# mkocabas/EpipolarPose

Measured on NVIDIA H100. Metric: multi-view samples/sec (4-view 256x256, bs32), higher is better.
Workload: dtype f16x3 (fp32 operands split into two fp16 planes, 3-pass error-compensated wgmma f16, f32 accumulate: fp32-grade results)

## Files before the change

### epipolarpose_b200/_lib.py

```python
import ctypes
import os

HERE = os.path.dirname(os.path.abspath(__file__))
LIB_PATH = os.environ.get("EPB_LIB_PATH") or os.path.join(HERE, "libepb.so")

EPB_MAX_TAPS = 64
EPB_JPEG_DESC_BYTES = 8192
EPB_JPEG_PLAN_LEN = 10
EPB_JPEG_EVENTS = 6
EPB_JPEG_STATS = 7

c_int, c_i64, c_f, c_d, c_p = (ctypes.c_int, ctypes.c_int64, ctypes.c_float,
                               ctypes.c_double, ctypes.c_void_p)


class ConvGeom(ctypes.Structure):
    _fields_ = [("N", c_int), ("Hi", c_int), ("Wi", c_int), ("Cin", c_int),
                ("Ho", c_int), ("Wo", c_int), ("Cout", c_int),
                ("Hp", c_int), ("Wp", c_int),
                ("os", c_int), ("ph", c_int), ("pw", c_int), ("is_", c_int),
                ("T", c_int),
                ("dh", c_int * EPB_MAX_TAPS), ("dw", c_int * EPB_MAX_TAPS),
                ("wt", c_int * EPB_MAX_TAPS), ("Tw", c_int),
                ("in_relu", c_int), ("accumulate", c_int), ("precision", c_int)]
# ... 25 lines not shown
    "epb_softargmax_fwd": (c_int, [c_p, c_int, c_int, c_int, c_int, c_int, c_int, c_p, c_p, c_p]),
    "epb_softargmax_bwd": (c_int, [c_p, c_int, c_int, c_int, c_int, c_int, c_int, c_p, c_p, c_p, c_p, c_p]),
    "epb_jointloss_fwd_bwd": (c_int, [c_p, c_p, c_p, c_int, c_int, c_int, c_f, c_p, c_p, c_p]),
    "epb_heatmap_joint_loss": (c_int, [c_p, c_p, c_p, c_int, c_int, c_f, c_p, c_p, c_p, c_int, c_int, c_f, c_f,
                                       c_p, c_p, c_p, c_p]),
    "epb_argmax2d": (c_int, [c_p, c_int, c_int, c_int, c_p, c_p, c_p, c_p]),
    "epb_final_preds": (c_int, [c_p, c_int, c_int, c_int, c_int, c_p, c_p, c_int, c_p, c_p, c_p]),
    "epb_patch_to_image": (c_int, [c_p, c_p, c_int, c_int, c_d, c_d, c_d, c_p, c_p]),
    "epb_triangulate": (c_int, [c_p, c_p, c_int, c_p, c_p, c_int, c_int, c_int, c_d, c_p, c_p, c_p]),
    "epb_triangulate_nview": (c_int, [c_p, c_int, c_p, c_int, c_int, c_int, c_p, c_p, c_p]),
    "epb_relative_pose": (c_int, [c_p, c_int, c_p, c_p, c_int, c_int, c_d, c_p, c_p, c_p, c_p, c_p, c_p,
                                  c_p]),
    "epb_project_labels": (c_int, [c_p, c_p, c_p, c_int, c_int, c_d, c_d, c_d, c_p, c_p, c_p]),
    "epb_h36m_eval": (c_int, [c_p, c_p, c_p, c_int, c_int, c_int, ctypes.c_uint32, c_d, c_p, c_p, c_p, c_p, c_p]),
    "epb_pose_normalize": (c_int, [c_p, c_p, c_int, c_int, c_int, c_p, c_p]),
    "epb_kmeans_workspace": (c_int, [c_int, c_int, c_int, ctypes.POINTER(c_i64)]),
    "epb_kmeans_fit": (c_int, [c_p, c_int, c_int, c_int, ctypes.c_uint64, c_int, c_int, c_p, c_p, c_p, c_p, c_p,
                               c_i64, ctypes.POINTER(c_d), ctypes.POINTER(ctypes.c_int32), c_p]),
    "epb_kmeans_assign": (c_int, [c_p, c_int, c_int, c_p, c_int, c_p, c_p, c_p]),
    "epb_add3": (c_int, [c_p, c_p, c_p, c_p, c_i64, c_p]),
    "epb_mask_scale": (c_int, [c_p, c_p, c_f, c_p, c_i64, c_p]),
    "epb_patch_sample": (c_int, [c_p, c_p, c_p, c_p, c_p, c_p, c_p, c_int, c_int, c_int, c_p, c_p, c_p]),
    "epb_patch_sample_occ": (c_int, [c_p] * 7 + [c_int, c_int, c_int] + [c_p] * 5 + [c_p]),
    "epb_patch_joints": (c_int, [c_p, c_p, c_p, c_int, c_int, c_d, c_d, c_d, c_int, c_p, c_p]),
    "epb_bn_finalize_scale": (c_int, [c_p, c_i64, c_int, c_p, c_p, c_f, c_f] + [c_p] * 12),
    "epb_softargmax_bwd_split": (c_int, [c_p] + [c_int] * 5 + [c_p] * 7),
    "epb_softargmax_flip_fwd": (c_int, [c_p] + [c_int] * 5 + [ctypes.POINTER(c_int), c_int, c_p, c_p]),
    "epb_act_scale": (c_int, [c_p, c_p, c_p, c_i64, c_int, c_p, c_p, c_p, c_p, c_p, c_p]),
    "epb_bn_act_split": (c_int, [c_p] * 8 + [c_int, c_i64, c_int, c_p, c_p, c_p, c_p]),
    "epb_bn_relu_maxpool_split": (c_int, [c_p] * 6 + [c_int] * 4 + [c_p]),
    "epb_im2col_split": (c_int, [c_p] * 3 + [c_int] * 11 + [c_p]),
    "epb_split16": (c_int, [c_p, ctypes.c_longlong, c_p, c_p, c_p, c_p]),
    "epb_split16_batch": (c_int, [c_p, c_int, ctypes.c_longlong, c_p, c_p]),
    "epb_conv16_fprop": (c_int, [ctypes.POINTER(ConvGeom)] + [c_p] * 8),
    "epb_conv16_wgrad": (c_int, [ctypes.POINTER(ConvGeom)] + [c_p] * 6 + [ctypes.c_longlong, c_p]),
    "epb_conv16_fprop_splitk": (c_int, [ctypes.POINTER(ConvGeom)] + [c_p] * 7 + [c_int, c_p, ctypes.c_longlong,
                                                                               c_p]),
    "epb_conv16_splits": (c_int, [ctypes.POINTER(ConvGeom), ctypes.POINTER(c_int),
                                  ctypes.POINTER(ctypes.c_longlong)]),
    "epb_bn_bwd_reduce_mx": (c_int, [c_p] * 7 + [c_int, c_i64, c_int, c_p, c_p, c_p]),
    "epb_bn_bwd_apply_split": (c_int, [c_p] * 8 + [c_int, c_p, c_p, c_i64, c_int] + [c_p] * 6),
    "epb_bn_bwd_split": (c_int, [c_p] * 9 + [c_int, c_i64, c_int] + [c_p] * 6),
    "epb_avgpool_split": (c_int, [c_p, c_p, c_p, c_int, c_int, c_int, c_p]),
    "epb_sumsq": (c_int, [c_p, c_i64, c_p, c_p]),
    "epb_clip_scale": (c_int, [c_p, c_i64, c_p, c_d, c_p]),
    "epb_adam_step": (c_int, [c_p, c_p, c_p, c_p, c_i64, c_f, c_f, c_f, c_f, c_f, c_int, c_f, c_p]),
    "epb_sgd_step": (c_int, [c_p, c_p, c_p, c_i64, c_f, c_f, c_f, c_int, c_int, c_f, c_p]),
    "epb_adam_step_dev": (c_int, [c_p, c_p, c_p, c_p, c_i64, c_p, c_p, c_p]),
    "epb_sgd_step_dev": (c_int, [c_p, c_p, c_p, c_i64, c_p, c_p, c_p]),
    "epb_jpeg_parse": (c_int, [c_p, c_p, c_int, c_p, c_p, c_p, c_p, c_p]),
    "epb_jpeg_decode": (c_int, [c_p, c_p, c_p, c_int, c_p, c_p, c_i64, c_p, c_p, c_p, c_p, c_p, c_p, c_p]),
    "epb_softargmax_flip_lse_fwd": (c_int, [c_p] + [c_int] * 5 + [ctypes.POINTER(c_int), c_int, c_p, c_p, c_p]),
    "epb_triangulate_robust": (c_int, [c_p, c_int, c_p, c_p, c_int, c_int, c_int, c_d, c_p, c_p, c_p, c_p, c_p]),
}

EXPORTS = tuple(_PROTOS)


class EpbError(RuntimeError):
    pass


_lib = None


def lib():
    global _lib
    if _lib is None:
        if not os.path.exists(LIB_PATH):
            raise EpbError("libepb.so not built (%s); run `python -c 'import __graft_entry__ as g; "
                           "g.build()'`. There is no CPU fallback." % LIB_PATH)
        L = ctypes.CDLL(LIB_PATH)
        for name, (res, args) in _PROTOS.items():
            fn = getattr(L, name)
            fn.restype = res
            fn.argtypes = args
        _lib = L
    return _lib


def check(rc):
    if rc != 0:
        raise EpbError("libepb call failed (%d): %s" % (rc, lib().epb_last_error().decode()))


def call(name, *args):
    check(getattr(lib(), name)(*args))
```

### epipolarpose_b200/csrc/core.cu

```cuda
#include "common.cuh"
#include <string.h>
#include <mutex>
#include <vector>

static thread_local char g_err[512] = "";

void epb_set_error(const char* fmt, ...) {
  va_list ap;
  va_start(ap, fmt);
  vsnprintf(g_err, sizeof(g_err), fmt, ap);
  va_end(ap);
}

extern "C" __attribute__((visibility("default"))) int epb_version(void) { return 100; }
extern "C" __attribute__((visibility("default"))) const char* epb_last_error(void) { return g_err; }

extern "C" __attribute__((visibility("default"))) int epb_device_check(void) {
  int n = 0;
  cudaError_t e = cudaGetDeviceCount(&n);
  if (e != cudaSuccess || n == 0) {
    epb_set_error("no CUDA device: %s", cudaGetErrorString(e));
    cudaGetLastError();
    return EPB_ENOGPU;
  }
  int dev = 0, major = 0;
  EPB_CUDA(cudaGetDevice(&dev));
  EPB_CUDA(cudaDeviceGetAttribute(&major, cudaDevAttrComputeCapabilityMajor, dev));
  if (major != 9) {
    epb_set_error("device %d has compute capability %d.x; libepb.so is built for sm_90a only", dev, major);
    return EPB_ENOGPU;
  }
  return EPB_OK;
}

struct WsEntry { int kind, dev; cudaStream_t st; void* p; size_t cap; };
static std::mutex g_ws_mu;
static std::vector<WsEntry> g_ws;

int epb_workspace(int kind, size_t bytes, cudaStream_t st, void** out) {
  int dev = 0;
  EPB_CUDA(cudaGetDevice(&dev));
  std::lock_guard<std::mutex> lock(g_ws_mu);
  WsEntry* e = nullptr;
  for (auto& w : g_ws)
    if (w.kind == kind && w.dev == dev && w.st == st) { e = &w; break; }
  if (e && e->cap >= bytes) {
    *out = e->p;
    return EPB_OK;
  }
  cudaStreamCaptureStatus cs = cudaStreamCaptureStatusNone;
  EPB_CUDA(cudaStreamIsCapturing(st, &cs));
  if (cs != cudaStreamCaptureStatusNone) {
    epb_set_error("internal scratch (kind %d) would have to grow to %zu bytes during CUDA graph "
                  "capture: run one eager step of the same shape first", kind, bytes);
    return EPB_EINVAL;
  }
  size_t cap = bytes < 4096 ? 4096 : bytes;
  void* p = nullptr;
  EPB_CUDA(cudaMalloc(&p, cap));
  EPB_CUDA(cudaMemsetAsync(p, 0, cap, st));
  if (e) { e->p = p; e->cap = cap; }
  else g_ws.push_back({kind, dev, st, p, cap});
  *out = p;
  return EPB_OK;
}
```

### epipolarpose_b200/lib/core/function.py

```python
import logging
import time

import numpy as np
import torch

from ..utils.img_utils import (self_supervision_device,
                               trans_coords_from_patch_to_org_3d_batch)
from .integral_loss import get_joint_location_coords_flip, get_result_func, joint_location_result_from_coords
from ..utils.utils import AverageMeter
from ..dataset.deferred import assemble_batch, cat_meta, is_deferred

logger = logging.getLogger(__name__)


def loader_batch(data):
    if is_deferred(data):
        return assemble_batch(data)
    if isinstance(data, dict) and 'cam_1' in data and 'cam_2' in data:
        a, b = data['cam_1'], data['cam_2']
        return (torch.cat([a[0], b[0]]), torch.cat([a[1], b[1]]), torch.cat([a[2], b[2]]),
                cat_meta(a[3], b[3]))
    return data


class _fused_head:

    def __init__(self, model):
        net = getattr(model, "module", model)
        self.net = net if hasattr(net, "fused_head_gradient") else None

    def __enter__(self):
        if self.net is not None:
            self.prev, self.net.fused_head_gradient = self.net.fused_head_gradient, True

    def __exit__(self, *exc):
        if self.net is not None:
            self.net.fused_head_gradient = self.prev


def _online_tri(config):
    train = getattr(config, 'TRAIN', None)
    return bool(train is not None and getattr(train, 'ONLINE_TRIANGULATION', False))


def _estimate_extrinsics(config):
    train = getattr(config, 'TRAIN', None)
    est = bool(train is not None and getattr(train, 'ESTIMATE_EXTRINSICS', False))
    if est and not _online_tri(config):
        raise ValueError("TRAIN.ESTIMATE_EXTRINSICS needs TRAIN.ONLINE_TRIANGULATION")
    return est


def online_epipolar_loss(criterion, preds, meta, method="iterative", estimate_extrinsics=False):
    from .integral_loss import softmax_integral_tensor, _WeightedLossFn
    from ..utils.img_utils import (patch_to_image_device, triangulate_device,
                                   labels_from_global_coords_device,
                                   labels_estimated_extrinsics_device)
    J = criterion.num_joints
    W, H = preds.shape[-1], preds.shape[-2]
    D = preds.shape[-3] // J
    coords = softmax_integral_tensor(preds, J, True, W, H, D)
    with torch.no_grad():
        kps = patch_to_image_device(coords.detach(), meta)
        if estimate_extrinsics:
            label, weight = labels_estimated_extrinsics_device(kps, meta, method)
        else:
            X = triangulate_device(kps, meta, method)
            label, weight = labels_from_global_coords_device(X, meta)
    return _WeightedLossFn.apply(coords, label, weight, criterion._kind, criterion.size_average,
                                 criterion.norm)


class GraphedTrainStep:

    def __init__(self, model, criterion, optimizer, online=False, method="iterative",
                 estimate_extrinsics=False):
        if isinstance(model, torch.nn.DataParallel) and len(model.device_ids) == 1:
            model = model.module
        self.model, self.criterion, self.optimizer = model, criterion, optimizer
        self.online, self.method = online, method
        if estimate_extrinsics and not online:
            raise ValueError("estimate_extrinsics needs online=True")
        self.estimate_extrinsics = bool(estimate_extrinsics)
        self.graph = None
        self.key = None
        self.warm_key = None
        self.failed = False
        self.calls = 0
        self.copy_stream, self.pending, self.stage_next = None, None, 0
        self.assemble_stream, self.staged = None, None
        self.stream = torch.cuda.Stream() if torch.cuda.is_available() else None

    def eager_step(self, x, label, weight, geom):
        if self.stream is None:
            return self._eager(x, label, weight, geom)
        cur = torch.cuda.current_stream()
        self.stream.wait_stream(cur)
        with torch.cuda.stream(self.stream):
            out = self._eager(x, label, weight, geom)
        cur.wait_stream(self.stream)
        return out

    def _eager(self, x, label, weight, geom):
        self.optimizer.zero_grad()
        with _fused_head(self.model):
            preds = self.model(x)
        if self.online:
            loss = online_epipolar_loss(self.criterion, preds, {"_packed": geom}, self.method,
                                        self.estimate_extrinsics)
        else:
            loss = self.criterion(preds, label, weight)
        loss.backward()
        self.optimizer.step()
        return loss.detach()

    def prefetch(self, batch_data):
        if self.graph is None or not torch.cuda.is_available() or batch_data.is_cuda:
            return
        if tuple(batch_data.shape) != tuple(self.sx.shape):
            return
        if self.copy_stream is None:
            self.copy_stream = torch.cuda.Stream()
            self.stage = [torch.empty_like(self.sx) for _ in range(2)]
            self.stage_evt = [torch.cuda.Event() for _ in range(2)]
            self.stage_free = [None, None]
        k = self.stage_next
        with torch.cuda.stream(self.copy_stream):
            if self.stage_free[k] is not None:
                self.copy_stream.wait_event(self.stage_free[k])
            self.stage[k].copy_(batch_data, non_blocking=True)
            self.stage_evt[k].record(self.copy_stream)
        self.pending = (batch_data, k)
        self.stage_next = 1 - k

    def stage_batch(self, batch):
        if self.graph is None or not torch.cuda.is_available() or not is_deferred(batch):
            return
        if self.assemble_stream is None:
            self.assemble_stream = torch.cuda.Stream()
        with torch.cuda.stream(self.assemble_stream):
            out = assemble_batch(batch)
            ev = torch.cuda.Event()
            ev.record(self.assemble_stream)
        self.staged = (batch, out, ev)
# ... 6 lines not shown
        cur.wait_event(staged[2])
        for t in staged[1][:3]:
            t.record_stream(cur)
        return staged[1]

    def _load_input(self, batch_data):
        if self.pending is not None and self.pending[0] is batch_data:
            k = self.pending[1]
            self.pending = None
            cur = torch.cuda.current_stream()
            cur.wait_event(self.stage_evt[k])
            self.sx.copy_(self.stage[k], non_blocking=True)
            ev = torch.cuda.Event()
            ev.record(cur)
            self.stage_free[k] = ev
        else:
            self.sx.copy_(batch_data, non_blocking=True)

    def __call__(self, batch_data, label=None, weight=None, meta=None):
        dev = next(self.model.parameters()).device
        B = batch_data.shape[0]
        geom = None
        if self.online:
            from ..utils.img_utils import pack_meta
            geom = pack_meta(meta, B, dev, self.estimate_extrinsics)
        key = (tuple(batch_data.shape), self.online, self.estimate_extrinsics)
        self.calls += 1
        if self.graph is not None and key == self.key:
            self._load_input(batch_data)
            if self.online:
                for k in self.sgeom:
                    self.sgeom[k].copy_(geom[k], non_blocking=True)
            else:
                self.slabel.copy_(label, non_blocking=True)
                self.sweight.copy_(weight, non_blocking=True)
            if hasattr(self.optimizer, "sync_hyper"):
                self.optimizer.sync_hyper()
            self.graph.replay()
            return self.sloss
        x = batch_data.to(dev, non_blocking=True)
        if not self.online:
            label, weight = label.to(dev, non_blocking=True), weight.to(dev, non_blocking=True)
        if self.graph is not None or self.failed or not torch.cuda.is_available() \
                or self.warm_key != key:
            self.warm_key = key
            return self.eager_step(x, label, weight, geom)
        sx = x.clone()
        sgeom = {k: v.clone() for k, v in geom.items()} if self.online else None
        slabel = label.clone() if not self.online else None
        sweight = weight.clone() if not self.online else None
        if hasattr(self.optimizer, "sync_hyper"):
            self.optimizer.sync_hyper()
        torch.cuda.synchronize()
        graph = torch.cuda.CUDAGraph()
        self.optimizer.zero_grad(set_to_none=True)
        try:
            with torch.cuda.graph(graph, stream=self.stream):
                sloss = self._eager(sx, slabel, sweight, sgeom)
        except Exception as e:
            logger.warning("CUDA-graph capture of the training step failed (%s); running eagerly", e)
            self.failed = True
            torch.cuda.synchronize()
            self.optimizer.zero_grad(set_to_none=True)
            return self.eager_step(x, label, weight, geom)
        self.sx, self.sgeom, self.slabel, self.sweight, self.sloss = sx, sgeom, slabel, sweight, sloss
        self.graph, self.key = graph, key
        self.graph.replay()
        return self.sloss


def _graph_capable(model, criterion, optimizer):
    from ..utils.utils import _FlatOptimizer
    if not hasattr(criterion, '_kind') or not isinstance(optimizer, _FlatOptimizer):
        return False
    if isinstance(model, torch.nn.DataParallel) and len(model.device_ids) != 1:
        return False
    return True


def train_integral(config, train_loader, model, criterion, optimizer, epoch):
    batch_time = AverageMeter()
    data_time = AverageMeter()
    losses = AverageMeter()
    model.train()
    online = _online_tri(config)
    method = getattr(config.TRAIN, 'TRIANGULATION_METHOD', 'iterative') if online else None
    estimate = _estimate_extrinsics(config)
    pending = []
    use_graph = bool(getattr(config.TRAIN, 'CUDA_GRAPH', True)) and \
        _graph_capable(model, criterion, optimizer)
    stepper = getattr(model, '_epb_graphed_step', None)
    if use_graph and (stepper is None or stepper.optimizer is not optimizer
                      or stepper.criterion is not criterion or stepper.online != online
                      or stepper.estimate_extrinsics != estimate):
        stepper = GraphedTrainStep(model, criterion, optimizer, online, method, estimate)
        model._epb_graphed_step = stepper
    end = time.time()
    it = iter(train_loader)
    nxt = next(it, None)
    i = -1
    while nxt is not None:
        data, i = nxt, i + 1
        nxt = next(it, None)
        data_time.update(time.time() - end)
        batch_data, batch_label, batch_label_weight, meta = \
            stepper.take(data) if use_graph else loader_batch(data)
        batch_size = batch_data.size(0)
        if use_graph:
            if stepper.pending is None and stepper.graph is not None:
                stepper.prefetch(batch_data)
            loss = stepper(batch_data, batch_label, batch_label_weight, meta)
# ... 175 lines not shown
```

### epipolarpose_b200/net.py

```python
import torch

from . import ops as _default_ops

BN_MOMENTUM = 0.1
BN_EPS = 1e-5

RESNET_SPEC = {18: ("basic", [2, 2, 2, 2]), 34: ("basic", [3, 4, 6, 3]),
               50: ("bottleneck", [3, 4, 6, 3]), 101: ("bottleneck", [3, 4, 23, 3]),
               152: ("bottleneck", [3, 8, 36, 3])}


def _pad(c, m):
    return (c + m - 1) // m * m


class Conv:

    def __init__(self, name, kind, cin, cout, k, stride, pad, opad=0, bias=False):
        self.name, self.kind = name, kind
        self.cin, self.cout, self.k, self.stride, self.pad, self.opad = cin, cout, k, stride, pad, opad
        self.bias = bias
        self.cin_p = _pad(cin, 4)
        self.cout_p = _pad(cout, 4)
        self._gcache = {}
# ... 442 lines not shown
        depth = None
        if plan.fc is not None:
            tr, th, tw = S["trunk"]
            assert th == plan.pool_k and tw == plan.pool_k, "AvgPool(k) -> 1x1 expected"
            pooled = self._new(N, 1, 1, 2048)
            ops.avgpool(tr, pooled, N, th * tw, 2048)
            depth, _, _ = self._conv_fwd(plan.fc, pooled, N, 1, 1, packed(plan.fc),
                                         bias=params["depth_fc.bias"])
            S["fc"] = pooled
        return logits, depth, (S if save else None)

    def _bn_bwd(self, st, dy, z, y_out, relu, params, grads):
        ops = self.ops
        C = st.C
        M = z.numel() // C
        gs = getattr(self, "_gs", None)
        sums = gs["bsum"][st.name] if gs is not None else \
            torch.zeros(2 * C, device=self.dev, dtype=torch.float64)
        ops.bn_bwd_reduce(dy, z, y_out, st.scale, st.shift, st.mean, st.invstd, relu, M, C, sums)
        dz = torch.empty_like(z)
        ops.bn_bwd_apply(dy, z, y_out, st.scale, st.shift, st.mean, st.invstd,
                         params[st.name + ".weight"], relu, sums, M, C, dz,
                         grads[st.name + ".weight"], grads[st.name + ".bias"])
        return dz

    def _stage_done(self, k):
        if k in self._stages_done:
            return
        self._stages_done.add(k)
        batch = self._gs["batches"][k]
        side = self._side
        if side is None:
            if batch is not None:
                self.ops.pack_weight_batch(batch)
            if self._on_stage is not None:
                self._on_stage(k)
            return
        side.wait_stream(torch.cuda.current_stream())
        with torch.cuda.stream(side):
            if batch is not None:
                self.ops.pack_weight_batch(batch)
            if self._on_stage is not None:
                self._on_stage(k)

    def backward(self, S, dlogits, ddepth, params, grads, on_stage=None):
        ops, plan = self.ops, self.plan
        N = S["N"]
        anchor = dlogits if dlogits is not None else self._head.planes
        self.dev = anchor.device
        import os
        self._side, self._keep = None, []
        if anchor.is_cuda and os.environ.get("EPB_OVERLAP_WGRAD", "1") != "0":
            if getattr(self, "_side_stream", None) is None:
                self._side_stream = torch.cuda.Stream()
            self._side = self._side_stream
        self._gs = self._grad_state(grads)
        self._gs["flat"].zero_()
        self._gs["sums"].zero_()
        self._on_stage, self._stages_done = on_stage, set()
        try:
            self._backward(S, dlogits, ddepth, params, grads)
            for k in range(len(STAGES)):
                self._stage_done(k)
        finally:
            if self._side is not None:
                torch.cuda.current_stream().wait_stream(self._side)
            self._side, self._keep, self._gs, self._on_stage = None, [], None, None

    def _backward(self, S, dlogits, ddepth, params, grads):
        ops, plan = self.ops, self.plan
        N = S["N"]

        def wd_of(conv):
            return S["packed"][conv.name][1]

        fin = plan.final
        src, aff, h, w = S["final"]
        Ho, Wo = fin.out_hw(h, w)
        gb = grads[fin.name + ".bias"]
        if fin.cout_p != fin.cout:
            tmp = torch.empty(fin.cout_p, device=self.dev)
            ops.colsum(dlogits, N * Ho * Wo, fin.cout_p, tmp)
            gb.copy_(tmp[:fin.cout])
        else:
            ops.colsum(dlogits, N * Ho * Wo, fin.cout_p, gb)
        self._conv_wgrad(fin, src, dlogits, N, h, w, grads[fin.name + ".weight"], affine=aff)
        dcur = self._conv_dgrad(fin, dlogits, N, h, w, wd_of(fin))
        for (conv, (bname, C)), (dsrc, daff, z, dh, dw) in zip(reversed(plan.deconvs),
                                                               reversed(S["deconv"])):
            st = S["bn"][bname]
            dz = self._bn_bwd(st, dcur, z, None, 1, params, grads)
            if conv.bias:
                oh, ow = conv.out_hw(dh, dw)
                ops.colsum(dz, N * oh * ow, conv.cout_p, grads[conv.name + ".bias"])
            self._conv_wgrad(conv, dsrc, dz, N, dh, dw, grads[conv.name + ".weight"], affine=daff)
            dcur = self._conv_dgrad(conv, dz, N, dh, dw, wd_of(conv))
        if plan.fc is not None and ddepth is not None:
            tr, th, tw = S["trunk"]
            dd = ddepth.reshape(N, 1, 1, -1).contiguous()
            ops.colsum(dd, N, plan.fc.cout_p, grads["depth_fc.bias"])
            self._conv_wgrad(plan.fc, S["fc"], dd, N, 1, 1, grads["depth_fc.weight"])
            dpool = self._conv_dgrad(plan.fc, dd, N, 1, 1, wd_of(plan.fc))
            ops.avgpool_bwd(dpool, dcur, N, th * tw, 2048, 1)
        self._stage_done(0)
        prev_stage = None
        for blk, rec in zip(reversed(plan.blocks), reversed(S["blocks"])):
            sk = stage_of(blk["name"])
# ... 39 lines not shown
```

### epipolarpose_b200/net16.py

```python
import os

import torch

from . import net as _net
from .net import BN_EPS, BN_MOMENTUM, Conv, _BNState

IMG_SCALE = 16.0
STEM_KPAD16 = 192
WGRAD_WS_FLOATS = 48 << 20


def supported(plan):
    convs = [c for c in plan.all_convs() if c is not plan.stem and c is not plan.final
             and c is not plan.fc]
    ok = all(c.cin % 64 == 0 and c.cout % 64 == 0 for c in convs)
    ok = ok and plan.final.cin % 64 == 0
    ok = ok and not any(c.bias for c, _ in plan.deconvs)
    return ok


class Engine16(_net.Engine):

    def __init__(self, plan, ops=None):
        super().__init__(plan, precision=3, ops=ops)
# ... 50 lines not shown
        packed = self._pack_weights(params)
        w16 = self._split_weights(packed)
        bn = state["bn"] if state is not None else {}
        for name, C in plan.all_bns():
            if name not in bn:
                bn[name] = self._bn_eval(name, C, params)
                continue
            ops.bn_eval_affine(C, params[name + ".weight"], params[name + ".bias"],
                               params[name + ".running_mean"], params[name + ".running_var"],
                               BN_EPS, bn[name].scale, bn[name].shift)
        fin = plan.final
        fbias = state["fbias"] if state is not None else torch.zeros(fin.cout_p, device=dev)
        fbias[:fin.cout].copy_(params[fin.name + ".bias"])
        return {"packed": packed, "w16": w16, "bn": bn, "fbias": fbias}

    def _conv_fwd16(self, conv, x, x_sc, N, H, W, w16, bias=None, stats=None, splitk=False):
        ops = self.ops
        Ho, Wo = conv.out_hw(H, W)
        geoms = self._geoms(conv, "f", N, H, W)
        need_zero = any(g is None for g in geoms)
        out = (torch.zeros if need_zero else torch.empty)(
            (N, Ho, Wo, conv.cout_p), device=self.dev, dtype=torch.float32)
        for g in geoms:
            if g is None:
                continue
            g.in_relu, g.accumulate = 0, 0
            if splitk:
                splits, n = ops.conv16_splits(g)
                ws = self._consts()["ws"]
                if n > ws.numel():
                    ws = torch.empty(n, device=self.dev, dtype=torch.float32)
                ops.conv16_fprop_splitk(g, x, x_sc, w16[0], w16[1], out, bias, stats, splits, ws)
            else:
                ops.conv16_fprop(g, x, x_sc, w16[0], w16[1], out, bias, stats)
        return out, Ho, Wo

    def _conv_dgrad16(self, conv, dz, dz_sc, N, H, W, wd16, accumulate_into=None):
        ops = self.ops
        geoms = self._geoms(conv, "d", N, H, W)
        if accumulate_into is not None:
            din = accumulate_into
        else:
            need_zero = any(g is None for g in geoms)
            din = (torch.zeros if need_zero else torch.empty)(
                (N, H, W, conv.cin_p), device=self.dev, dtype=torch.float32)
        for g in geoms:
            if g is None:
                continue
            g.in_relu = 0
            g.accumulate = 1 if accumulate_into is not None else 0
            ops.conv16_fprop(g, dz, dz_sc, wd16[0], wd16[1], din, None, None)
        return din

    def _conv_wgrad16(self, conv, x, x_sc, dz, dz_sc, N, H, W):
        ops = self.ops
        dwp = self._gs["dwp"][conv.name]
        ws = self._consts()["ws"]

        def run():
            for g in self._geoms(conv, "f", N, H, W):
                if g is None:
                    continue
                g.in_relu, g.accumulate = 0, 0
                ops.conv16_wgrad(g, x, x_sc, dz, dz_sc, dwp, ws)

        side = getattr(self, "_side", None)
        if side is None:
            run()
            return
        main = torch.cuda.current_stream()
        side.wait_stream(main)
        self._keep.append((x, dz, dz_sc))
        with torch.cuda.stream(side):
            run()

    def _bn_bwd16(self, st, dy, z, mask_bits, relu, params, grads, dy_masked=None):
        ops = self.ops
        C = st.C
        M = z.numel() // C
        dz = self._half(*z.shape)
        dz_sc = torch.empty(2, device=self.dev, dtype=torch.float32)
        ops.bn_bwd_split(dy, z, None, st.scale, st.shift, st.mean, st.invstd,
                         params[st.name + ".weight"], relu, M, C, dz, dz_sc, dy_masked,
                         grads[st.name + ".weight"], grads[st.name + ".bias"], mask_bits=mask_bits)
        return dz, dz_sc

    def forward(self, x_nchw, params, training=True, save=True, prepared=None):
        ops, plan = self.ops, self.plan
        infer = prepared is not None
        if infer and (training or save):
            raise ValueError("a forward on prepared weights is an inference forward (training=False, save=False)")
        self.dev = x_nchw.device
        N, _, H, W = x_nchw.shape
        cst = self._consts()
        S = {"N": N, "H": H, "W": W, "bn": {}, "blocks": []}
        bns = plan.all_bns()
        offs, tot = {}, 0
        for name, C in bns:
            offs[name] = tot
            tot += 2 * C
        stats_all = torch.zeros(tot, device=self.dev, dtype=torch.float64)
        scs = torch.empty((len(bns) + 1, 4), device=self.dev, dtype=torch.float32)
        sc_slot = [0]

        def new_sc():
            sc_slot[0] += 1
            return scs[sc_slot[0] - 1]

        def stats_of(name, C):
            return stats_all[offs[name]:offs[name] + 2 * C]

        def bn(name, C, M, sc=None, group2=(None, None, None), res_sc=None):
            if training:
                fused = None if sc is None else group2 + (res_sc, sc)
                st = self._bn_train(name, C, stats_of(name, C), M, params, None, act_scale=fused)
            else:
                st = prepared["bn"][name] if infer else self._bn_eval(name, C, params)
                if sc is not None:
                    ops.act_scale(stats_of(name, C), st.scale, st.shift, M, C, *group2, res_sc, sc)
            S["bn"][name] = st
            return st

        self._nbt_tick = []

# ... 95 lines not shown
        depth = None
        if plan.fc is not None:
            tr, tr_sc, th, tw = S["trunk"]
            assert th == plan.pool_k and tw == plan.pool_k, "AvgPool(k) -> 1x1 expected"
            pooled = torch.empty((N, 1, 1, 2048), device=self.dev, dtype=torch.float32)
            ops.avgpool_split(tr, tr_sc, pooled, N, th * tw, 2048)
            depth, _, _ = self._conv_fwd(plan.fc, pooled, N, 1, 1, S["packed"][plan.fc.name][0],
                                         bias=params["depth_fc.bias"])
            S["fc"] = pooled
        tick, self._nbt_tick = self._nbt_tick, None
        if tick:
            torch._foreach_add_(tick, 1)
        return logits, depth, (S if save else None)

    def backward(self, S, dlogits, ddepth, params, grads, on_stage=None, head=None):
        self._head = head
        try:
            super().backward(S, dlogits, ddepth, params, grads, on_stage=on_stage)
        finally:
            self._head = None

    def takes_logit_sink(self):
        fin = self.plan.final
        return self.plan.fc is None and fin.cout_p == fin.cout and fin.cout_p % 64 == 0

    def _backward(self, S, dlogits, ddepth, params, grads):
        ops, plan = self.ops, self.plan
        N = S["N"]

        def wd16(conv):
            return S["w16"][conv.name][1]

        fin = plan.final
        src, aff, h, w = S["final"]
        Ho, Wo = fin.out_hw(h, w)
        gb = grads[fin.name + ".bias"]
        head = getattr(self, "_head", None)
        if head is not None:
            gb.copy_(head.dbias)
        elif fin.cout_p != fin.cout:
            tmp = torch.empty(fin.cout_p, device=self.dev)
            ops.colsum(dlogits, N * Ho * Wo, fin.cout_p, tmp)
            gb.copy_(tmp[:fin.cout])
        else:
            ops.colsum(dlogits, N * Ho * Wo, fin.cout_p, gb)
        if fin.cout_p % 64 == 0:
            if head is not None:
                dl16, dl_sc = head.planes, head.sc
            else:
                dl16 = self._half(N, Ho, Wo, fin.cout_p)
                dl_sc = torch.empty(2, device=self.dev, dtype=torch.float32)
                ops.split16(dlogits.reshape(-1), dl16.reshape(-1), dl_sc, self._consts()["amax1"])
            fsrc, fsrc_sc = S["final16"]
            self._conv_wgrad16(fin, fsrc, fsrc_sc, dl16, dl_sc, N, h, w)
            dcur = self._conv_dgrad16(fin, dl16, dl_sc, N, h, w, wd16(fin))
        else:
            self._conv_wgrad(fin, src, dlogits, N, h, w, grads[fin.name + ".weight"], affine=aff)
            dcur = self._conv_dgrad(fin, dlogits, N, h, w, S["packed"][fin.name][1])
        for (conv, (bname, C)), (dsrc, dsrc_sc, z, dh, dw) in zip(reversed(plan.deconvs),
                                                                  reversed(S["deconv"])):
            st = S["bn"][bname]
            dz, dsc = self._bn_bwd16(st, dcur, z, None, 1, params, grads)
            self._conv_wgrad16(conv, dsrc, dsrc_sc, dz, dsc, N, dh, dw)
            dcur = self._conv_dgrad16(conv, dz, dsc, N, dh, dw, wd16(conv))
        if plan.fc is not None and ddepth is not None:
            tr, tr_sc, th, tw = S["trunk"]
            dd = ddepth.reshape(N, 1, 1, -1).contiguous()
            ops.colsum(dd, N, plan.fc.cout_p, grads["depth_fc.bias"])
            self._conv_wgrad(plan.fc, S["fc"], dd, N, 1, 1, grads["depth_fc.weight"])
            dpool = self._conv_dgrad(plan.fc, dd, N, 1, 1, S["packed"][plan.fc.name][1])
            ops.avgpool_bwd(dpool, dcur, N, th * tw, 2048, 1)
        self._stage_done(0)
        prev_stage = None
        for blk, rec in zip(reversed(plan.blocks), reversed(S["blocks"])):
            sk = _net.stage_of(blk["name"])
            if prev_stage is not None and sk != prev_stage:
                self._stage_done(prev_stage)
            prev_stage = sk
            (out, _), (xin, xin_sc), h, w = rec["out"], rec["in"], rec["h"], rec["w"]
            nconv = len(blk["convs"])
            mask = rec["mask"]
            down = blk["down"]
            if down:
                dconv, (dname, dC) = down
                dzd, dzd_sc = self._bn_bwd16(S["bn"][dname], dcur, rec["zd"], mask, 0, params, grads)
            g = dcur
            for ci in range(nconv - 1, -1, -1):
                conv = blk["convs"][ci]
                st = S["bn"][blk["bns"][ci][0]]
                z = rec["z"][ci]
                if ci == nconv - 1:
                    dz, dsc = self._bn_bwd16(st, dcur, z, mask, 0, params, grads,
                                             dy_masked=None if down else dcur)
                else:
                    dz, dsc = self._bn_bwd16(st, g, z, None, 1, params, grads)
                hh, ww = rec["hw"][ci]
                xop, xop_sc = (xin, xin_sc) if ci == 0 else rec["a"][ci - 1]
                self._conv_wgrad16(conv, xop, xop_sc, dz, dsc, N, hh, ww)
                if ci == 0 and not down:
                    g = self._conv_dgrad16(conv, dz, dsc, N, hh, ww, wd16(conv), accumulate_into=dcur)
                else:
                    g = self._conv_dgrad16(conv, dz, dsc, N, hh, ww, wd16(conv))
            if down:
                self._conv_wgrad16(dconv, xin, xin_sc, dzd, dzd_sc, N, h, w)
                self._conv_dgrad16(dconv, dzd, dzd_sc, N, h, w, wd16(dconv), accumulate_into=g)
            dcur = g
        col, z0, argidx, H1, W1, H2, W2 = S["stem"]
        gpool = torch.empty((N, H1, W1, 64), device=self.dev, dtype=torch.float32)
        ops.maxpool_bwd(dcur, argidx, gpool, N, H1, W1, 64)
        dz0, dsc0 = self._bn_bwd16(S["bn"]["bn1"], gpool, z0, None, 1, params, grads)
        self._conv_wgrad16(self.stem_col, col, self._consts()["img_sc"], dz0, dsc0, N, H1, W1)
```

### epipolarpose_b200/ops.py

```python
import ctypes

import torch

from . import _lib
from ._lib import ConvGeom

launches = 0

_KERNELS_PER_CALL = {
    "epb_softargmax_fwd": 2, "epb_softargmax_flip_fwd": 2, "epb_softargmax_flip_lse_fwd": 2, "epb_bn_bwd_apply": 2, "epb_colsum": 3,
    "epb_split16_batch": 3, "epb_split16": 3, "epb_bn_bwd_apply_split": 2, "epb_conv16_wgrad": 2,
    "epb_bn_bwd_reduce_mx": 2, "epb_bn_bwd_split": 3, "epb_softargmax_bwd_split": 3,
    "epb_patch_sample": 2, "epb_patch_sample_occ": 2, "epb_jpeg_decode": 14,
}


def _stream():
    return ctypes.c_void_p(torch.cuda.current_stream().cuda_stream)


def _p(t, dtype=torch.float32):
    if t is None:
        return None
    if not t.is_cuda:
        raise _lib.EpbError("tensor must live on a CUDA device (no CPU fallback)")
    if t.dtype != dtype:
        raise _lib.EpbError("expected dtype %s, got %s" % (dtype, t.dtype))
    if t.device.index != torch.cuda.current_device():
        raise _lib.EpbError("tensor lives on cuda:%d but the current device is cuda:%d (wrap the call in "
                            "torch.cuda.device(tensor.device))" % (t.device.index, torch.cuda.current_device()))
    if not t.is_contiguous():
        raise _lib.EpbError("tensor must be contiguous")
    return ctypes.c_void_p(t.data_ptr())


def _call(name, *args):
    global launches
    _lib.call(name, *args)
    launches += _KERNELS_PER_CALL.get(name, 1)


def device_check():
    _lib.call("epb_device_check")



def make_geom(N, Hi, Wi, Cin, Ho, Wo, Cout, Hp, Wp, os, ph, pw, is_, taps, Tw,
              in_relu=0, accumulate=0, precision=0):
    g = ConvGeom()
    g.N, g.Hi, g.Wi, g.Cin = N, Hi, Wi, Cin
    g.Ho, g.Wo, g.Cout = Ho, Wo, Cout
    g.Hp, g.Wp, g.os, g.ph, g.pw, g.is_ = Hp, Wp, os, ph, pw, is_
    g.T = len(taps)
# ... 383 lines not shown

def triangulate_nview(u, stride_u, P, NT, V, J, X, status):
    _call("epb_triangulate_nview", _p(u, torch.float64), stride_u, _p(P, torch.float64), NT, V, J,
          _p(X, torch.float64), _p(status, torch.int32), _stream())


def triangulate_robust(u, stride_u, P, w, NT, V, J, threshold_px, X, inliers, resid, status):
    _call("epb_triangulate_robust", _p(u, torch.float64), stride_u, _p(P, torch.float64),
          _p(w, torch.float64), NT, V, J, float(threshold_px), _p(X, torch.float64),
          _p(inliers, torch.int32), _p(resid, torch.float64), _p(status, torch.int32), _stream())


def relative_pose(u, stride_u, intr, box, B, J, rect3d_w, Pa, Pb, cam, inliers, status, diag=None):
    _call("epb_relative_pose", _p(u, torch.float64), stride_u, _p(intr, torch.float64),
          _p(box, torch.float64), B, J, float(rect3d_w), _p(Pa, torch.float64), _p(Pb, torch.float64),
          _p(cam, torch.float64), _p(inliers, torch.int32), _p(status, torch.int32),
          _p(diag, torch.int32), _stream())


def project_labels(X, cam, box, B, J, patch_w, patch_h, rect3d_w, label, weight):
    _call("epb_project_labels", _p(X, torch.float64), _p(cam, torch.float64),
          _p(box, torch.float64), B, J, float(patch_w), float(patch_h), float(rect3d_w),
          _p(label), _p(weight), _stream())


def sumsq(x, n, total):
    _call("epb_sumsq", _p(x), n, _p(total, torch.float64), _stream())


def clip_scale(x, n, total, max_norm):
    _call("epb_clip_scale", _p(x), n, _p(total, torch.float64), float(max_norm), _stream())


def adam_step(param, grad, exp_avg, exp_avg_sq, n, lr, beta1, beta2, eps, weight_decay, step,
              grad_scale=1.0):
    _call("epb_adam_step", _p(param), _p(grad), _p(exp_avg), _p(exp_avg_sq), n, lr, beta1, beta2,
          eps, weight_decay, step, grad_scale, _stream())


def sgd_step(param, grad, buf, n, lr, momentum, weight_decay, nesterov, first_step,
             grad_scale=1.0):
    _call("epb_sgd_step", _p(param), _p(grad), _p(buf), n, lr, momentum, weight_decay,
          int(nesterov), int(first_step), grad_scale, _stream())


def adam_step_dev(param, grad, exp_avg, exp_avg_sq, n, hyper, step_dev):
    _call("epb_adam_step_dev", _p(param), _p(grad), _p(exp_avg), _p(exp_avg_sq), n, _p(hyper),
          _p(step_dev, torch.int32), _stream())


def sgd_step_dev(param, grad, buf, n, hyper, step_dev):
    _call("epb_sgd_step_dev", _p(param), _p(grad), _p(buf), n, _p(hyper),
          _p(step_dev, torch.int32), _stream())
```

### include/epb.h

```cpp
#ifndef EPB_H_
#define EPB_H_

#include <stdint.h>

#ifdef __cplusplus
extern "C" {
#endif

#define EPB_OK 0
#define EPB_EINVAL (-1)
#define EPB_ECUDA (-2)
#define EPB_ENOGPU (-3)

#define EPB_MAX_TAPS 64

typedef void* epb_stream_t;

int epb_version(void);
const char* epb_last_error(void);
int epb_device_check(void);

typedef struct {
  int N, Hi, Wi, Cin;
  int Ho, Wo, Cout;
// ... 205 lines not shown
                   int64_t ws_bytes, double* inertia_host, int32_t* n_iter_host, epb_stream_t stream);
int epb_kmeans_assign(const double* x, int N, int d, const double* centroids, int k, int32_t* labels,
                      double* dist2, epb_stream_t stream);

int epb_add3(const float* a, const float* b, const float* c, float* out, int64_t n, epb_stream_t stream);
int epb_mask_scale(const float* x, const uint8_t* mask, float scale, float* out, int64_t n,
                   epb_stream_t stream);

int epb_sumsq(const float* x, int64_t n, double* total, epb_stream_t stream);
int epb_clip_scale(float* x, int64_t n, const double* total, double max_norm, epb_stream_t stream);

int epb_patch_sample(const uint8_t* img_base, const int64_t* img_off, const int32_t* img_hwp,
                     const double* box, const int32_t* flip, const float* color,
                     const double* mean_std_host, int B, int patch_w, int patch_h, float* out,
                     double* trans, epb_stream_t stream);
int epb_patch_sample_occ(const uint8_t* img_base, const int64_t* img_off, const int32_t* img_hwp,
                         const double* box, const int32_t* flip, const float* color,
                         const double* mean_std_host, int B, int patch_w, int patch_h,
                         const uint8_t* occ_base, const int64_t* occ_desc, const int32_t* occ_count,
                         float* out, double* trans, epb_stream_t stream);
int epb_patch_joints(const double* joints, const double* box, const double* trans, int B, int J,
                     double patch_w, double patch_h, double rect_3d_w, int depth_in_image,
                     double* label, epb_stream_t stream);

#define EPB_JPEG_OK 0
#define EPB_JPEG_UNSUPPORTED 1
#define EPB_JPEG_MALFORMED 2
#define EPB_JPEG_DESC_BYTES 8192
#define EPB_JPEG_PLAN_LEN 10
#define EPB_JPEG_EVENTS 6
#define EPB_JPEG_STATS 7
int epb_jpeg_parse(const uint8_t* const* blobs_host, const int64_t* lens_host, int B, void* desc_host,
                   int32_t* status_host, int32_t* hw_host, int64_t* out_off_host, int64_t* plan_host);
int epb_jpeg_decode(const uint8_t* blob_base, const int64_t* blob_off, const void* desc, int B,
                    const int64_t* plan_host, void* ws, int64_t ws_bytes, uint8_t* out_base,
                    const int64_t* out_off, const int32_t* out_hwp, int32_t* status, int32_t* stats,
                    void* const* events_host, epb_stream_t stream);

int epb_adam_step(float* param, const float* grad, float* exp_avg,
                  float* exp_avg_sq, int64_t n, float lr, float beta1,
                  float beta2, float eps, float weight_decay, int step,
                  float grad_scale, epb_stream_t stream);
int epb_sgd_step(float* param, const float* grad, float* momentum_buf, int64_t n,
                 float lr, float momentum, float weight_decay, int nesterov,
                 int first_step, float grad_scale, epb_stream_t stream);

int epb_adam_step_dev(float* param, const float* grad, float* exp_avg,
                      float* exp_avg_sq, int64_t n, const float* hyper,
                      const int* step_dev, epb_stream_t stream);
int epb_sgd_step_dev(float* param, const float* grad, float* momentum_buf,
                     int64_t n, const float* hyper, const int* step_dev,
                     epb_stream_t stream);

#ifdef __cplusplus
}
#endif
#endif
```

Baseline: 482.1.

## Prioritize dgrad critical path over side-stream wgrad in captured training graph

Gives the main training stream high priority and the side wgrad stream low priority, then re-instantiates the captured CUDA graph with node priorities honored. Each wgrad launch now waits on an event recorded before the dgrad instead of the whole main stream, and is issued after the dgrad. The aim is to let the critical-path dgrad kernels run ahead while wgrad fills idle SMs. It adds a custom graph exec wrapper, which is a new lifetime and compatibility risk, and a debug helper that lists graph kernel nodes.

```diff
diff --git a/epipolarpose_b200/_lib.py b/epipolarpose_b200/_lib.py
--- a/epipolarpose_b200/_lib.py
+++ b/epipolarpose_b200/_lib.py
@@ -101,6 +101,11 @@
     "epb_jpeg_decode": (c_int, [c_p, c_p, c_p, c_int, c_p, c_p, c_i64, c_p, c_p, c_p, c_p, c_p, c_p, c_p]),
     "epb_softargmax_flip_lse_fwd": (c_int, [c_p] + [c_int] * 5 + [ctypes.POINTER(c_int), c_int, c_p, c_p, c_p]),
     "epb_triangulate_robust": (c_int, [c_p, c_int, c_p, c_p, c_int, c_int, c_int, c_d, c_p, c_p, c_p, c_p, c_p]),
+    "epb_graph_instantiate": (c_int, [c_p, ctypes.POINTER(c_p)]),
+    "epb_graph_launch": (c_int, [c_p, c_p]),
+    "epb_graph_exec_destroy": (c_int, [c_p]),
+    "epb_graph_kernel_nodes": (c_int, [c_p, c_int, ctypes.POINTER(c_int), ctypes.POINTER(ctypes.c_char_p),
+                                       ctypes.POINTER(c_int)]),
 }
 
 EXPORTS = tuple(_PROTOS)
diff --git a/epipolarpose_b200/csrc/core.cu b/epipolarpose_b200/csrc/core.cu
--- a/epipolarpose_b200/csrc/core.cu
+++ b/epipolarpose_b200/csrc/core.cu
@@ -64,3 +64,57 @@
   *out = p;
   return EPB_OK;
 }
+
+#define EPB_EXPORT extern "C" __attribute__((visibility("default")))
+
+EPB_EXPORT int epb_graph_instantiate(void* graph, void** exec) {
+  EPB_CHECK_ARG(graph && exec);
+  cudaGraphExec_t g = nullptr;
+  EPB_CUDA(cudaGraphInstantiateWithFlags(&g, static_cast<cudaGraph_t>(graph),
+                                         cudaGraphInstantiateFlagAutoFreeOnLaunch |
+                                             cudaGraphInstantiateFlagUseNodePriority));
+  *exec = g;
+  return EPB_OK;
+}
+
+EPB_EXPORT int epb_graph_launch(void* exec, epb_stream_t stream) {
+  EPB_CHECK_ARG(exec);
+  EPB_CUDA(cudaGraphLaunch(static_cast<cudaGraphExec_t>(exec), as_stream(stream)));
+  return EPB_OK;
+}
+
+EPB_EXPORT int epb_graph_exec_destroy(void* exec) {
+  EPB_CHECK_ARG(exec);
+  EPB_CUDA(cudaGraphExecDestroy(static_cast<cudaGraphExec_t>(exec)));
+  return EPB_OK;
+}
+
+EPB_EXPORT int epb_graph_kernel_nodes(void* graph, int cap, int* prio, const char** names, int* n) {
+  EPB_CHECK_ARG(graph && n && cap >= 0 && (cap == 0 || (prio && names)));
+  cudaGraph_t g = static_cast<cudaGraph_t>(graph);
+  size_t count = 0;
+  EPB_CUDA(cudaGraphGetNodes(g, nullptr, &count));
+  std::vector<cudaGraphNode_t> nodes(count);
+  EPB_CUDA(cudaGraphGetNodes(g, nodes.data(), &count));
+  int k = 0;
+  for (cudaGraphNode_t node : nodes) {
+    cudaGraphNodeType t;
+    EPB_CUDA(cudaGraphNodeGetType(node, &t));
+    if (t != cudaGraphNodeTypeKernel) continue;
+    if (k < cap) {
+      cudaLaunchAttributeValue v;
+      EPB_CUDA(cudaGraphKernelNodeGetAttribute(node, cudaLaunchAttributePriority, &v));
+      prio[k] = v.priority;
+      names[k] = "";
+      cudaKernelNodeParams p;
+      const char* name = nullptr;
+      if (cudaGraphKernelNodeGetParams(node, &p) == cudaSuccess && cudaFuncGetName(&name, p.func) == cudaSuccess &&
+          name)
+        names[k] = name;
+      cudaGetLastError();
+    }
+    ++k;
+  }
+  *n = k;
+  return EPB_OK;
+}
diff --git a/epipolarpose_b200/lib/core/function.py b/epipolarpose_b200/lib/core/function.py
--- a/epipolarpose_b200/lib/core/function.py
+++ b/epipolarpose_b200/lib/core/function.py
@@ -9,6 +9,7 @@
 from .integral_loss import get_joint_location_coords_flip, get_result_func, joint_location_result_from_coords
 from ..utils.utils import AverageMeter
 from ..dataset.deferred import assemble_batch, cat_meta, is_deferred
+from epipolarpose_b200 import ops as _ops
 
 logger = logging.getLogger(__name__)
 
@@ -89,7 +90,8 @@
         self.calls = 0
         self.copy_stream, self.pending, self.stage_next = None, None, 0
         self.assemble_stream, self.staged = None, None
-        self.stream = torch.cuda.Stream() if torch.cuda.is_available() else None
+        self.stream = torch.cuda.Stream(priority=torch.cuda.Stream.priority_range()[1]) \
+            if torch.cuda.is_available() else None
 
     def eager_step(self, x, label, weight, geom):
         if self.stream is None:
@@ -202,11 +204,12 @@
         if hasattr(self.optimizer, "sync_hyper"):
             self.optimizer.sync_hyper()
         torch.cuda.synchronize()
-        graph = torch.cuda.CUDAGraph()
+        graph = torch.cuda.CUDAGraph(keep_graph=True)
         self.optimizer.zero_grad(set_to_none=True)
         try:
             with torch.cuda.graph(graph, stream=self.stream):
                 sloss = self._eager(sx, slabel, sweight, sgeom)
+            graph = _ops.PriorityGraph(graph)
         except Exception as e:
             logger.warning("CUDA-graph capture of the training step failed (%s); running eagerly", e)
             self.failed = True
diff --git a/epipolarpose_b200/net.py b/epipolarpose_b200/net.py
--- a/epipolarpose_b200/net.py
+++ b/epipolarpose_b200/net.py
@@ -518,7 +518,7 @@
         self._side, self._keep = None, []
         if anchor.is_cuda and os.environ.get("EPB_OVERLAP_WGRAD", "1") != "0":
             if getattr(self, "_side_stream", None) is None:
-                self._side_stream = torch.cuda.Stream()
+                self._side_stream = torch.cuda.Stream(priority=torch.cuda.Stream.priority_range()[0])
             self._side = self._side_stream
         self._gs = self._grad_state(grads)
         self._gs["flat"].zero_()
diff --git a/epipolarpose_b200/net16.py b/epipolarpose_b200/net16.py
--- a/epipolarpose_b200/net16.py
+++ b/epipolarpose_b200/net16.py
@@ -126,7 +126,14 @@
             ops.conv16_fprop(g, dz, dz_sc, wd16[0], wd16[1], din, None, None)
         return din
 
-    def _conv_wgrad16(self, conv, x, x_sc, dz, dz_sc, N, H, W):
+    def _operands_ready(self):
+        if getattr(self, "_side", None) is None:
+            return None
+        ev = torch.cuda.Event()
+        ev.record()
+        return ev
+
+    def _conv_wgrad16(self, conv, x, x_sc, dz, dz_sc, N, H, W, ready=None):
         ops = self.ops
         dwp = self._gs["dwp"][conv.name]
         ws = self._consts()["ws"]
@@ -142,8 +149,10 @@
         if side is None:
             run()
             return
-        main = torch.cuda.current_stream()
-        side.wait_stream(main)
+        if ready is not None:
+            side.wait_event(ready)
+        else:
+            side.wait_stream(torch.cuda.current_stream())
         self._keep.append((x, dz, dz_sc))
         with torch.cuda.stream(side):
             run()
@@ -345,8 +354,9 @@
                 dl_sc = torch.empty(2, device=self.dev, dtype=torch.float32)
                 ops.split16(dlogits.reshape(-1), dl16.reshape(-1), dl_sc, self._consts()["amax1"])
             fsrc, fsrc_sc = S["final16"]
-            self._conv_wgrad16(fin, fsrc, fsrc_sc, dl16, dl_sc, N, h, w)
+            ready = self._operands_ready()
             dcur = self._conv_dgrad16(fin, dl16, dl_sc, N, h, w, wd16(fin))
+            self._conv_wgrad16(fin, fsrc, fsrc_sc, dl16, dl_sc, N, h, w, ready)
         else:
             self._conv_wgrad(fin, src, dlogits, N, h, w, grads[fin.name + ".weight"], affine=aff)
             dcur = self._conv_dgrad(fin, dlogits, N, h, w, S["packed"][fin.name][1])
@@ -354,8 +364,9 @@
                                                                   reversed(S["deconv"])):
             st = S["bn"][bname]
             dz, dsc = self._bn_bwd16(st, dcur, z, None, 1, params, grads)
-            self._conv_wgrad16(conv, dsrc, dsrc_sc, dz, dsc, N, dh, dw)
+            ready = self._operands_ready()
             dcur = self._conv_dgrad16(conv, dz, dsc, N, dh, dw, wd16(conv))
+            self._conv_wgrad16(conv, dsrc, dsrc_sc, dz, dsc, N, dh, dw, ready)
         if plan.fc is not None and ddepth is not None:
             tr, tr_sc, th, tw = S["trunk"]
             dd = ddepth.reshape(N, 1, 1, -1).contiguous()
@@ -389,14 +400,16 @@
                     dz, dsc = self._bn_bwd16(st, g, z, None, 1, params, grads)
                 hh, ww = rec["hw"][ci]
                 xop, xop_sc = (xin, xin_sc) if ci == 0 else rec["a"][ci - 1]
-                self._conv_wgrad16(conv, xop, xop_sc, dz, dsc, N, hh, ww)
+                ready = self._operands_ready()
                 if ci == 0 and not down:
                     g = self._conv_dgrad16(conv, dz, dsc, N, hh, ww, wd16(conv), accumulate_into=dcur)
                 else:
                     g = self._conv_dgrad16(conv, dz, dsc, N, hh, ww, wd16(conv))
+                self._conv_wgrad16(conv, xop, xop_sc, dz, dsc, N, hh, ww, ready)
             if down:
-                self._conv_wgrad16(dconv, xin, xin_sc, dzd, dzd_sc, N, h, w)
+                ready = self._operands_ready()
                 self._conv_dgrad16(dconv, dzd, dzd_sc, N, h, w, wd16(dconv), accumulate_into=g)
+                self._conv_wgrad16(dconv, xin, xin_sc, dzd, dzd_sc, N, h, w, ready)
             dcur = g
         col, z0, argidx, H1, W1, H2, W2 = S["stem"]
         gpool = torch.empty((N, H1, W1, 64), device=self.dev, dtype=torch.float32)
diff --git a/epipolarpose_b200/ops.py b/epipolarpose_b200/ops.py
--- a/epipolarpose_b200/ops.py
+++ b/epipolarpose_b200/ops.py
@@ -1,4 +1,5 @@
 import ctypes
+import weakref
 
 import torch
 
@@ -488,3 +489,26 @@
 def sgd_step_dev(param, grad, buf, n, hyper, step_dev):
     _call("epb_sgd_step_dev", _p(param), _p(grad), _p(buf), n, _p(hyper),
           _p(step_dev, torch.int32), _stream())
+
+
+
+class PriorityGraph:
+
+    def __init__(self, graph):
+        self.graph = graph
+        h = ctypes.c_void_p()
+        _lib.call("epb_graph_instantiate", ctypes.c_void_p(graph.raw_cuda_graph()), ctypes.byref(h))
+        self._h = h
+        self._fin = weakref.finalize(self, _lib.lib().epb_graph_exec_destroy, h)
+        self._fin.atexit = False
+
+    def replay(self):
+        _lib.call("epb_graph_launch", self._h, _stream())
+
+
+def graph_kernel_nodes(graph):
+    raw, n = ctypes.c_void_p(graph.raw_cuda_graph()), ctypes.c_int()
+    _lib.call("epb_graph_kernel_nodes", raw, 0, None, None, ctypes.byref(n))
+    prio, names = (ctypes.c_int * n.value)(), (ctypes.c_char_p * n.value)()
+    _lib.call("epb_graph_kernel_nodes", raw, n.value, prio, names, ctypes.byref(n))
+    return [(prio[i], (names[i] or b"").decode()) for i in range(n.value)]
diff --git a/include/epb.h b/include/epb.h
--- a/include/epb.h
+++ b/include/epb.h
@@ -281,6 +281,11 @@
                      int64_t n, const float* hyper, const int* step_dev,
                      epb_stream_t stream);
 
+int epb_graph_instantiate(void* graph, void** exec);
+int epb_graph_launch(void* exec, epb_stream_t stream);
+int epb_graph_exec_destroy(void* exec);
+int epb_graph_kernel_nodes(void* graph, int cap, int* prio, const char** names, int* n);
+
 #ifdef __cplusplus
 }
 #endif
```

Result: faster. 489.9 (median of 6 runs) (+1.6%).
